# lRomul/sensorium

Hardware: AMD Instinct MI355X
Metric: training clips/sec/GPU (DwiseNeuro fwd+bwd, B=32 T=32 36x64) at 1/2/4/8 GPUs (higher is better)
Workload: dtype bf16

## Files before the change

### include/dwn.h

```cpp
#ifndef DWN_H_
#define DWN_H_
#include <stddef.h>
#include <stdint.h>

#ifdef __cplusplus
extern "C" {
#endif

#define DWN_ABI_VERSION 7
#define DWN_F32 0
#define DWN_BF16 1
#define DWN_F32_AUTO 0
#define DWN_F32_NATIVE 1
#define DWN_F32_SPLIT3 2
#define DWN_BN_EVAL 0
#define DWN_BN_TRAIN 1
#define DWN_BN_FROZEN 2
#define DWN_NREP 32

#define DWN_LD_PLAIN 0
#define DWN_LD_PE 1
#define DWN_LD_BNACT 2
#define DWN_LD_AFFINE2 3
#define DWN_LD_DY3 4
#define DWN_LD_GATE 5
#define DWN_LD_CAT1 6

typedef struct dwn_load_desc {
    const void* p;
    const void* q;
    long long ld;
    const float* v1;
    const float* v2;
    const float* v3;
    const float* v4;
    const float* v5;
    const float* gate;
    const float* gate2;
    int gate_ld;
    int rows_per_sample;
    int act;
    const float* pe_t;
    const float* pe_h;
    const float* pe_w;
    int pT, pH, pW;
    int pe_ld;
    long long ld2;
    int cat_c1, cat_c2;
} dwn_load_desc;

#define DWN_EPI_STORE 0
#define DWN_EPI_READOUT 1
#define DWN_EPI_DG 2
#define DWN_EPI_STORE_CAT 3
#define DWN_EPI_DH3 4

typedef struct dwn_gemm_nn_args {
    dwn_load_desc a;
    int a_kind;
    const void* b; long long ldb;
    void* c; long long ldc;
    int M, N, K;
    int groups;
    double* stats;
    int f32_split;
    int stat_nchan;
    int epi;
    const float* bias; float sp_beta; float* out_nct; int Tn; int n_valid;
    const void* y3; long long ldy3; const float* s3; const float* t3; float* dg; int dg_ld; int rows_per_sample;
    const void* a2; long long a2_ld; int K1;
    long long b_sample_stride; int b_rows_per_sample;
    const float* gate3; const float* dps3; const float* coef3; int coef3_ld;
    int variant;
    const float* sp_beta_dev;
} dwn_gemm_nn_args;
#define DWN_NN_AUTO 0
#define DWN_NN_XL128 1
#define DWN_NN_XL256 2
#define DWN_NN_TILE128 3
#define DWN_NN_KD 4

typedef struct dwn_gemm_tn_args {
    dwn_load_desc p; int p_kind;
    dwn_load_desc q; int q_kind;
    int M, R, Cc;
    float* dw; long long lddw;
    int groups;
    int rows_per_split; int nsplit;
    int R_load;
    int rows_per_sample; int splits_per_sample; long long dw_sample_stride;
    int overwrite;
    int dw_f64;
} dwn_gemm_tn_args;

typedef struct dwn_dw_spatial_fwd_args {
    dwn_load_desc in;
    const float* w;
    void* out;
    int planes, Hin, Win, Hout, Wout, C, stride, ks;
    double* stats;
    int rows_band;
    int impl;
    const void* a0; long long a0_ld; const void* w1; int Cin;
} dwn_dw_spatial_fwd_args;

typedef struct dwn_dw_spatial_bwd_args {
    dwn_load_desc dy;
    dwn_load_desc y1;
    const float* w;
    void* dh1;
    float* dw;
    int planes, Hin, Win, Hout, Wout, C, stride, ks;
    double* stats;
    int rows_band;
    int impl;
    const void* a0; long long a0_ld; const void* w1; int Cin;
} dwn_dw_spatial_bwd_args;

typedef struct dwn_dw_temporal_fwd_args {
    dwn_load_desc in;
    const float* w;
    void* out;
    int B, T, HW, C, kt;
    double* stats;
    const float* z_scale; const float* z_shift; long long* pooled;
} dwn_dw_temporal_fwd_args;

typedef struct dwn_dw_temporal_bwd_args {
    dwn_load_desc dy; int dy_kind;
    dwn_load_desc y2;
    const float* w;
    void* dh2;
    float* dw;
    int B, T, HW, C, kt;
    double* stats;
} dwn_dw_temporal_bwd_args;

typedef struct dwn_bn {
    const float* gamma; const float* beta;
    float* running_mean; float* running_var; long long* num_batches_tracked;
    float* coef;
    float* dgamma; float* dbeta;
} dwn_bn;

typedef struct dwn_stem_args {
    int dtype, training, B, Cin, C0; long long S;
    float eps, momentum;
    const float* x;
    const float* w;
    dwn_bn bn;
    const float *pe_t, *pe_h, *pe_w;
    int T, H, W;
    void* y0;
    void* out;
    const void* dout;
    float* dw;
    void* ws; size_t ws_bytes;
    double* xmom;
} dwn_stem_args;

typedef struct dwn_stem_input_grad_args {
    int dtype, training, B, Cin, C0; long long S;
    const float* w;
// ... 481 lines not shown
```

### sensorium_amd/_lib.py

```python
from __future__ import annotations

import ctypes as C
import os
from pathlib import Path

import torch

_HERE = Path(__file__).resolve().parent
DETERMINISTIC = os.environ.get("DWN_DETERMINISTIC", "0") == "1"
_LIB_NAME = "libdwiseneuro_hip_det.so" if DETERMINISTIC else "libdwiseneuro_hip.so"
LIB_PATH = Path(os.environ["DWN_LIB_PATH"]) if os.environ.get("DWN_LIB_PATH") else _HERE / "csrc" / _LIB_NAME

c_p = C.c_void_p
c_i = C.c_int
c_ll = C.c_longlong
c_f = C.c_float
c_d = C.c_double
c_sz = C.c_size_t

DWN_F32, DWN_BF16 = 0, 1
DWN_NREP = 32
LD_PLAIN, LD_PE, LD_BNACT, LD_AFFINE2, LD_DY3, LD_GATE, LD_CAT1 = 0, 1, 2, 3, 4, 5, 6
EPI_STORE, EPI_READOUT, EPI_DG, EPI_STORE_CAT, EPI_DH3 = 0, 1, 2, 3, 4
NN_AUTO, NN_XL128, NN_XL256, NN_TILE128, NN_KD = 0, 1, 2, 3, 4
F32_AUTO, F32_NATIVE, F32_SPLIT3 = 0, 1, 2
BN_EVAL, BN_TRAIN, BN_FROZEN = 0, 1, 2
FAMILIES = ("pw_fwd", "dws_fwd", "dwt_fwd", "se_pool", "pwl_fwd", "resid_fwd", "resid_bwd", "pwl_dgrad", "pwl_wgrad",
            "bn3_reduce", "dwt_bwd", "dws_bwd", "pw_dgrad", "pw_wgrad", "cortex_fwd", "cortex_bwd", "readout_fwd",
            "readout_bwd")


class LoadDesc(C.Structure):
    _fields_ = [("p", c_p), ("q", c_p), ("ld", c_ll), ("v1", c_p), ("v2", c_p), ("v3", c_p), ("v4", c_p),
                ("v5", c_p), ("gate", c_p), ("gate2", c_p), ("gate_ld", c_i), ("rows_per_sample", c_i),
                ("act", c_i), ("pe_t", c_p), ("pe_h", c_p), ("pe_w", c_p), ("pT", c_i), ("pH", c_i),
                ("pW", c_i), ("pe_ld", c_i), ("ld2", c_ll), ("cat_c1", c_i), ("cat_c2", c_i)]


class GemmNNArgs(C.Structure):
    _fields_ = [("a", LoadDesc), ("a_kind", c_i), ("b", c_p), ("ldb", c_ll), ("c", c_p), ("ldc", c_ll),
                ("M", c_i), ("N", c_i), ("K", c_i), ("groups", c_i), ("stats", c_p),
                ("f32_split", c_i), ("stat_nchan", c_i), ("epi", c_i), ("bias", c_p),
                ("sp_beta", c_f), ("out_nct", c_p), ("Tn", c_i), ("n_valid", c_i), ("y3", c_p), ("ldy3", c_ll),
                ("s3", c_p), ("t3", c_p), ("dg", c_p), ("dg_ld", c_i), ("rows_per_sample", c_i),
                ("a2", c_p), ("a2_ld", c_ll), ("K1", c_i), ("b_sample_stride", c_ll), ("b_rows_per_sample", c_i),
                ("gate3", c_p), ("dps3", c_p), ("coef3", c_p), ("coef3_ld", c_i), ("variant", c_i), ("sp_beta_dev", c_p)]


class GemmTNArgs(C.Structure):
    _fields_ = [("p", LoadDesc), ("p_kind", c_i), ("q", LoadDesc), ("q_kind", c_i), ("M", c_i), ("R", c_i),
                ("Cc", c_i), ("dw", c_p), ("lddw", c_ll), ("groups", c_i), ("rows_per_split", c_i),
                ("nsplit", c_i), ("R_load", c_i), ("rows_per_sample", c_i), ("splits_per_sample", c_i),
                ("dw_sample_stride", c_ll), ("overwrite", c_i), ("dw_f64", c_i)]


class DwSpatialFwdArgs(C.Structure):
    _fields_ = [("inp", LoadDesc), ("w", c_p), ("out", c_p), ("planes", c_i), ("Hin", c_i), ("Win", c_i),
                ("Hout", c_i), ("Wout", c_i), ("C", c_i), ("stride", c_i), ("ks", c_i), ("stats", c_p),
                ("rows_band", c_i), ("impl", c_i),
                ("a0", c_p), ("a0_ld", c_ll), ("w1", c_p), ("Cin", c_i)]


class DwSpatialBwdArgs(C.Structure):
    _fields_ = [("dy", LoadDesc), ("y1", LoadDesc), ("w", c_p), ("dh1", c_p), ("dw", c_p), ("planes", c_i),
                ("Hin", c_i), ("Win", c_i), ("Hout", c_i), ("Wout", c_i), ("C", c_i), ("stride", c_i),
                ("ks", c_i), ("stats", c_p), ("rows_band", c_i), ("impl", c_i),
                ("a0", c_p), ("a0_ld", c_ll), ("w1", c_p), ("Cin", c_i)]


class DwTemporalFwdArgs(C.Structure):
    _fields_ = [("inp", LoadDesc), ("w", c_p), ("out", c_p), ("B", c_i), ("T", c_i), ("HW", c_i), ("C", c_i),
                ("kt", c_i), ("stats", c_p), ("z_scale", c_p), ("z_shift", c_p), ("pooled", c_p)]


class DwTemporalBwdArgs(C.Structure):
    _fields_ = [("dy", LoadDesc), ("dy_kind", c_i), ("y2", LoadDesc), ("w", c_p), ("dh2", c_p), ("dw", c_p),
                ("B", c_i), ("T", c_i), ("HW", c_i), ("C", c_i), ("kt", c_i), ("stats", c_p)]


class BN(C.Structure):
    _fields_ = [("gamma", c_p), ("beta", c_p), ("running_mean", c_p), ("running_var", c_p),
                ("num_batches_tracked", c_p), ("coef", c_p), ("dgamma", c_p), ("dbeta", c_p)]


class StemArgs(C.Structure):
    _fields_ = [("dtype", c_i), ("training", c_i), ("B", c_i), ("Cin", c_i), ("C0", c_i), ("S", c_ll),
                ("eps", c_f), ("momentum", c_f), ("x", c_p), ("w", c_p), ("bn", BN),
                ("pe_t", c_p), ("pe_h", c_p), ("pe_w", c_p), ("T", c_i), ("H", c_i), ("W", c_i),
                ("y0", c_p), ("out", c_p),
                ("dout", c_p), ("dw", c_p), ("ws", c_p), ("ws_bytes", c_sz), ("xmom", c_p)]


class StemInputGradArgs(C.Structure):
    _fields_ = [("dtype", c_i), ("training", c_i), ("B", c_i), ("Cin", c_i), ("C0", c_i), ("S", c_ll),
                ("w", c_p), ("coef", c_p), ("dout", c_p), ("dx", c_p)]


class BlockArgs(C.Structure):
    _fields_ = [("dtype", c_i), ("training", c_i),
                ("B", c_i), ("T", c_i), ("Hin", c_i), ("Win", c_i), ("Hout", c_i), ("Wout", c_i), ("Cin", c_i),
                ("Cmid", c_i), ("Cout", c_i), ("stride", c_i), ("ks", c_i), ("kt", c_i), ("se_r", c_i),
                ("eps", c_f), ("momentum", c_f),
                ("x", c_p), ("out", c_p), ("y1", c_p), ("y2", c_p), ("y3", c_p), ("y4", c_p),
                ("z3", c_p), ("x_has_pe", c_i), ("a0", c_p),
                ("pe_t", c_p), ("pe_h", c_p), ("pe_w", c_p),
                ("out_pe_t", c_p), ("out_pe_h", c_p), ("out_pe_w", c_p),
                ("w_pw", c_p), ("w_dws", c_p), ("w_dwt", c_p), ("w_pwl", c_p), ("se_wr", c_p), ("se_br", c_p),
# ... 169 lines not shown
CORR_STAT_ROWS, CORR_TILE = 8, 16
CORR_MEAN, CORR_SUM = 0, 1
GABOR_GAUSSIAN, GABOR_NONE = 0, 1
BLUR_MAX_RADIUS, BLUR_TAPS_STRIDE, MOMENTS_CHUNK = 16, 33, 4096
MEI_STEP, MEI_PROJECT = 0, 1
MEI_CONTRAST_MAX, MEI_CONTRAST_FIXED = 0, 1
TRIAL_STATE_ROWS, TRIAL_SCORE_ROWS, TRIAL_SUMMARY, TRIAL_TILE = 17, 5, 8, 4
NOISE_BINARY, NOISE_SPARSE = 0, 1
STA_SUMMARY = 8
GAUSS_PARAMS, GAUSS_TABLE = 7, 16
PAIR_TOTAL, PAIR_SIGNAL, PAIR_NOISE = 0, 1, 2
PAIR_TILE, PAIR_KSTEP, PAIR_SUMMARY, PAIR_ROW_STATS = 64, 4, 8, 8
MIX_BOX, MIX_BLEND = 0, 1
VID_U8, VID_F32 = 0, 1

_STRUCTS = {
    "dwn_load_desc": LoadDesc, "dwn_gemm_nn_args": GemmNNArgs, "dwn_gemm_tn_args": GemmTNArgs,
    "dwn_dw_spatial_fwd_args": DwSpatialFwdArgs, "dwn_dw_spatial_bwd_args": DwSpatialBwdArgs,
    "dwn_dw_temporal_fwd_args": DwTemporalFwdArgs, "dwn_dw_temporal_bwd_args": DwTemporalBwdArgs,
    "dwn_bn": BN, "dwn_stem_args": StemArgs, "dwn_block_args": BlockArgs, "dwn_pool_args": PoolArgs,
    "dwn_cortex_args": CortexArgs, "dwn_readout_args": ReadoutArgs, "dwn_tensor_entry": TensorEntry,
    "dwn_clip_src": ClipSrc, "dwn_clip_desc": ClipDesc, "dwn_pw_bwd_args": PwBwdArgs,
    "dwn_dw_spatial_rc_fwd_args": DwSpatialRcFwdArgs, "dwn_stem_input_grad_args": StemInputGradArgs,
    "dwn_guarded_entry": GuardedEntry, "dwn_step_guard": StepGuard, "dwn_gaze_args": GazeArgs,
    "dwn_corr_args": CorrArgs, "dwn_gabor_args": GaborArgs, "dwn_modulator_args": ModulatorArgs,
    "dwn_blur3d_args": Blur3dArgs, "dwn_clip_moments_args": ClipMomentsArgs, "dwn_mei_update_args": MeiUpdateArgs,
    "dwn_trial_desc": TrialDesc, "dwn_trial_group": TrialGroup, "dwn_trial_score_args": TrialScoreArgs,
    "dwn_spatial_gain_args": SpatialGainArgs, "dwn_noise_args": NoiseArgs, "dwn_sta_args": StaArgs,
    "dwn_gauss2d_args": Gauss2dArgs, "dwn_gauss2d_profile_args": Gauss2dProfileArgs,
    "dwn_pair_seg": PairSeg, "dwn_pair_args": PairArgs, "dwn_pair_compare_args": PairCompareArgs,
}

_P = C.POINTER
SYMBOLS = {
    "dwn_abi_version": (c_i, []),
    "dwn_source_hash": (C.c_char_p, []),
    "dwn_sizeof": (c_i, [C.c_char_p]),
    "dwn_last_error": (C.c_char_p, []),
    "dwn_profile_enable": (c_i, [C.c_ulonglong, c_i]),
    "dwn_profile_collect": (c_i, [c_i, _P(c_d), _P(c_ll)]),
    "dwn_gemm_nn": (c_i, [_P(GemmNNArgs), c_i, c_i, c_p]),
    "dwn_gemm_tn": (c_i, [_P(GemmTNArgs), c_i, c_i, c_p]),
    "dwn_dw_spatial_fwd": (c_i, [_P(DwSpatialFwdArgs), c_i, c_i, c_p]),
    "dwn_dw_spatial_bwd": (c_i, [_P(DwSpatialBwdArgs), c_i, c_i, c_p]),
    "dwn_dw_spatial_bwd_rc_supported": (c_i, [_P(DwSpatialBwdArgs), c_i]),
    "dwn_dw_spatial_fwd_rc_supported": (c_i, [_P(DwSpatialFwdArgs), c_i]),
    "dwn_dw_temporal_fwd": (c_i, [_P(DwTemporalFwdArgs), c_i, c_i, c_p]),
    "dwn_dw_temporal_bwd": (c_i, [_P(DwTemporalBwdArgs), c_i, c_i, c_p]),
    "dwn_dw_temporal_wide_fwd": (c_i, [_P(DwTemporalFwdArgs), c_i, c_i, c_p]),
    "dwn_dw_temporal_wide_bwd": (c_i, [_P(DwTemporalBwdArgs), c_i, c_i, c_p]),
    "dwn_bn_finalize": (c_i, [c_p, c_i, c_d, _P(BN), c_i, c_i, c_f, c_f, c_i, c_p]),
    "dwn_bn_bwd_finalize": (c_i, [c_p, c_d, _P(BN), c_p, c_i, c_i, c_p]),
    "dwn_pack_weight": (c_i, [c_p, c_p, c_i, c_i, c_i, c_i, c_i, c_i, c_i, c_i, c_p]),
    "dwn_stem_workspace_bytes": (c_sz, [_P(StemArgs)]),
    "dwn_stem_forward": (c_i, [_P(StemArgs), c_i, c_p]),
    "dwn_stem_backward": (c_i, [_P(StemArgs), c_i, c_p]),
    "dwn_stem_input_grad": (c_i, [_P(StemInputGradArgs), c_i, c_p]),
    "dwn_stem_backward_input": (c_i, [_P(StemArgs), c_p, c_i, c_p]),
    "dwn_block_workspace_bytes": (c_sz, [_P(BlockArgs), c_i]),
    "dwn_block_forward": (c_i, [_P(BlockArgs), c_i, c_p]),
    "dwn_block_backward": (c_i, [_P(BlockArgs), c_i, c_p]),
    "dwn_block_forward_writes": (c_i, [_P(BlockArgs)]),
    "dwn_pool_forward": (c_i, [_P(PoolArgs), c_i, c_p]),
    "dwn_pool_backward": (c_i, [_P(PoolArgs), c_i, c_p]),
    "dwn_cortex_workspace_bytes": (c_sz, [_P(CortexArgs), c_i]),
    "dwn_cortex_forward": (c_i, [_P(CortexArgs), c_i, c_p]),
    "dwn_cortex_backward": (c_i, [_P(CortexArgs), c_i, c_p]),
    "dwn_readout_workspace_bytes": (c_sz, [_P(ReadoutArgs), c_i]),
    "dwn_readout_wt_bytes": (c_sz, [_P(ReadoutArgs)]),
    "dwn_readout_forward": (c_i, [_P(ReadoutArgs), c_i, c_p]),
    "dwn_readout_backward": (c_i, [_P(ReadoutArgs), c_i, c_p]),
    "dwn_poisson_loss_forward": (c_i, [c_p, c_p, c_p, c_ll, c_ll, c_f, c_p, c_i, c_p]),
    "dwn_poisson_loss_backward": (c_i, [c_p, c_p, c_p, c_p, c_ll, c_ll, c_f, c_p, c_i, c_p]),
    "dwn_f64_to_f32": (c_i, [c_p, c_p, c_i, c_i, c_p]),
    "dwn_adamw_ema_multi": (c_i, [c_p, c_i, c_i, c_d, c_d, c_d, c_d, c_d, c_ll, c_d, c_d, c_i, c_p]),
    "dwn_ema_lerp_multi": (c_i, [c_p, c_i, c_i, c_d, c_i, c_p]),
    "dwn_grad_guard_workspace_bytes": (c_sz, [c_i, c_i]),
    "dwn_grad_sumsq_multi": (c_i, [c_p, c_i, c_i, c_d, c_p, c_sz, c_p, c_i, c_p]),
    "dwn_step_guard_finalize": (c_i, [c_p, c_p, c_d, c_i, c_p, c_i, c_p, c_i, c_p]),
    "dwn_adamw_ema_multi_guarded": (c_i, [c_p, c_i, c_i, c_d, c_d, c_d, c_d, c_d, c_d, c_d, c_p, c_i, c_p]),
    "dwn_conv_pw_bn_stats_workspace_bytes": (c_sz, [c_i]),
    "dwn_conv_pw_bn_stats": (c_i, [c_p, c_ll, c_ll, c_p, c_i, c_i, _P(BN), c_f, c_f, c_p, c_p, c_sz, c_i, c_i, c_p]),
    "dwn_pw_bwd_fused_supported": (c_i, [c_i, c_ll, c_i, c_i]),
    "dwn_pw_backward_workspace_bytes": (c_sz, [c_i, c_i, c_i]),
    "dwn_pw_backward": (c_i, [_P(PwBwdArgs), c_i, c_i, c_p]),
    "dwn_dw_spatial_rc_blob_bytes": (c_sz, [c_i, c_i]),
    "dwn_dw_spatial_rc_prep": (c_i, [c_p, c_p, c_p, c_i, c_i, c_p, c_i, c_p]),
    "dwn_dw_spatial_rc_supported": (c_i, [c_i, c_i, c_i, c_i, c_i, c_i, c_i]),
    "dwn_dw_spatial_fwd_rc": (c_i, [_P(DwSpatialRcFwdArgs), c_i, c_p]),
    "dwn_assemble_inputs": (c_i, [c_p, c_i, c_i, c_i, c_i, c_i, c_i, c_f, c_p, c_i, c_p]),
    "dwn_assemble_targets": (c_i, [c_p, c_i, c_i, c_p, c_p, c_i, c_i, c_p, c_i, c_p]),
    "dwn_gaze_shift_forward": (c_i, [_P(GazeArgs), c_i, c_p]),
    "dwn_gaze_shift_backward": (c_i, [_P(GazeArgs), c_i, c_p]),
    "dwn_plane_mean": (c_i, [c_p, c_i, c_i, c_i, c_i, c_i, c_i, c_i, c_p, c_i, c_p]),
    "dwn_corr_ws_bytes": (c_sz, [_P(CorrArgs)]),
    "dwn_corr_moments": (c_i, [_P(CorrArgs), c_i, c_p]),
    "dwn_corr_loss_finalize": (c_i, [_P(CorrArgs), c_i, c_p]),
    "dwn_corr_loss_backward": (c_i, [_P(CorrArgs), c_i, c_p]),
    "dwn_gabor_workspace_bytes": (c_sz, [_P(GaborArgs)]),
    "dwn_gabor_forward": (c_i, [_P(GaborArgs), c_i, c_p]),
    "dwn_gabor_backward": (c_i, [_P(GaborArgs), c_i, c_p]),
    "dwn_modulator_ws_bytes": (c_sz, [_P(ModulatorArgs)]),
    "dwn_modulator_forward": (c_i, [_P(ModulatorArgs), c_i, c_p]),
    "dwn_modulator_backward": (c_i, [_P(ModulatorArgs), c_i, c_p]),
    "dwn_blur3d_ws_bytes": (c_sz, [_P(Blur3dArgs)]),
    "dwn_clip_moments_ws_bytes": (c_sz, [_P(ClipMomentsArgs)]),
    "dwn_blur3d": (c_i, [_P(Blur3dArgs), c_i, c_p]),
    "dwn_clip_moments": (c_i, [_P(ClipMomentsArgs), c_i, c_p]),
    "dwn_mei_update": (c_i, [_P(MeiUpdateArgs), c_i, c_p]),
    "dwn_trial_score_ws_bytes": (c_sz, [_P(TrialScoreArgs)]),
    "dwn_trial_moments": (c_i, [_P(TrialScoreArgs), c_i, c_p]),
    "dwn_trial_score_finalize": (c_i, [_P(TrialScoreArgs), c_i, c_p]),
    "dwn_spatial_gain_ws_bytes": (c_sz, [_P(SpatialGainArgs)]),
    "dwn_spatial_gain_forward": (c_i, [_P(SpatialGainArgs), c_i, c_p]),
    "dwn_spatial_gain_backward": (c_i, [_P(SpatialGainArgs), c_i, c_p]),
    "dwn_pair_ldz": (c_ll, [c_i]),
    "dwn_pair_state_bytes": (c_sz, [_P(PairArgs)]),
    "dwn_pair_ws_bytes": (c_sz, [_P(PairArgs)]),
    "dwn_pair_compare_ws_bytes": (c_sz, [_P(PairCompareArgs)]),
    "dwn_pair_stage": (c_i, [_P(PairArgs), c_i, c_p]),
    "dwn_pair_syrk": (c_i, [_P(PairArgs), c_i, c_p]),
    "dwn_pair_corr_finalize": (c_i, [_P(PairArgs), c_i, c_p]),
    "dwn_pair_compare": (c_i, [_P(PairCompareArgs), c_i, c_p]),
    "dwn_gauss2d_ws_bytes": (c_sz, [_P(Gauss2dArgs)]),
    "dwn_gauss2d_fit": (c_i, [_P(Gauss2dArgs), c_i, c_p]),
    "dwn_gauss2d_profile": (c_i, [_P(Gauss2dProfileArgs), c_i, c_p]),
    "dwn_noise_forward": (c_i, [_P(NoiseArgs), c_i, c_p]),
    "dwn_sta_state_bytes": (c_sz, [_P(StaArgs)]),
    "dwn_sta_ws_bytes": (c_sz, [_P(StaArgs)]),
    "dwn_sta_accumulate": (c_i, [_P(StaArgs), c_i, c_p]),
    "dwn_sta_finalize": (c_i, [_P(StaArgs), c_i, c_p]),
}


class DwnError(RuntimeError):
    pass


HASH_SRCS = ("dwn_api.hip", "dwn_gemm.hip", "dwn_gemm_nn_1.hip", "dwn_gemm_nn_2.hip", "dwn_gemm_nn_3.hip", "dwn_gemm_nn_4.hip", "dwn_gemm_nn_5.hip",
             "dwn_gemm_nn_6.hip", "dwn_gemm_tn.hip", "dwn_pw_bwd.hip", "dwn_gemm_xl.hip", "dwn_gemm_kd.hip", "dwn_dwconv.hip", "dwn_dwrc.hip",
             "dwn_dwbwd.hip", "dwn_dwfwd.hip", "dwn_elementwise.hip", "dwn_data.hip", "dwn_gaze.hip", "dwn_modulator.hip", "dwn_spatial.hip", "dwn_mei.hip", "dwn_rf_fit.hip", "dwn_pairwise.hip", "dwn_trial_score.hip", "dwn_rf.hip", "dwn_corr.hip", "dwn_stim.hip", "dwn_common.h", "dwn_internal.h",
             "dwn_kernels.h", "dwn_launch.h", "dwn_gemm_nn.h", "dwn_gain.h",
             "../../include/dwn.h")


def source_hash() -> str:
    import hashlib
    h = hashlib.sha256()
    for name in HASH_SRCS:
        h.update((_HERE / "csrc" / name).read_bytes())
    return h.hexdigest()[:16]


def _load():
    if not LIB_PATH.exists():
        raise ImportError(
            f"{LIB_PATH} is missing: build it with `python -c 'import __graft_entry__ as g; g.build()'` "
            f"(or `make -C {LIB_PATH.parent}`).  sensorium_amd has no fallback path.")
    lib = C.CDLL(str(LIB_PATH), mode=getattr(os, "RTLD_NOW", 2))
    ab = bool(os.environ.get("DWN_LIB_PATH"))
    for name, (restype, argtypes) in SYMBOLS.items():
        if ab and name in ("dwn_stem_input_grad", "dwn_stem_backward_input", "dwn_grad_guard_workspace_bytes", "dwn_grad_sumsq_multi",
                           "dwn_step_guard_finalize", "dwn_adamw_ema_multi_guarded", "dwn_dw_temporal_wide_fwd",
                           "dwn_dw_temporal_wide_bwd", "dwn_gaze_shift_forward", "dwn_gaze_shift_backward",
                           "dwn_plane_mean", "dwn_corr_ws_bytes", "dwn_corr_moments", "dwn_corr_loss_finalize",
                           "dwn_corr_loss_backward", "dwn_gabor_workspace_bytes", "dwn_gabor_forward",
                           "dwn_gabor_backward", "dwn_modulator_ws_bytes", "dwn_modulator_forward",
                           "dwn_modulator_backward", "dwn_blur3d_ws_bytes", "dwn_clip_moments_ws_bytes", "dwn_blur3d",
                           "dwn_clip_moments", "dwn_mei_update", "dwn_trial_score_ws_bytes", "dwn_trial_moments",
                           "dwn_trial_score_finalize", "dwn_spatial_gain_ws_bytes", "dwn_spatial_gain_forward",
                           "dwn_spatial_gain_backward", "dwn_noise_forward", "dwn_sta_state_bytes", "dwn_sta_ws_bytes",
                           "dwn_sta_accumulate", "dwn_sta_finalize", "dwn_gauss2d_ws_bytes", "dwn_gauss2d_fit",
                           "dwn_gauss2d_profile", "dwn_pair_ldz", "dwn_pair_state_bytes", "dwn_pair_ws_bytes",
                           "dwn_pair_compare_ws_bytes", "dwn_pair_stage", "dwn_pair_syrk", "dwn_pair_corr_finalize",
                           "dwn_pair_compare") and not hasattr(lib, name):
            continue
        fn = getattr(lib, name)
        fn.restype = restype
        fn.argtypes = argtypes
    if lib.dwn_abi_version() != 7 and not (ab and lib.dwn_abi_version() == 6):
        raise ImportError("libdwiseneuro_hip.so ABI version mismatch")
    built, have = lib.dwn_source_hash().decode(), source_hash()
    if built != have and not os.environ.get("DWN_LIB_PATH"):
        raise ImportError(f"{LIB_PATH.name} was built from other sources (binary {built}, tree {have}): rebuild it with "
                          f"`make -C {LIB_PATH.parent}` — binaries are not in git, so what runs must be what is committed")
    for cname, struct in _STRUCTS.items():
        n = lib.dwn_sizeof(cname.encode())
        if n != C.sizeof(struct) and not (ab and (0 < n < C.sizeof(struct) or cname in ("dwn_stem_input_grad_args", "dwn_guarded_entry", "dwn_step_guard", "dwn_gaze_args", "dwn_corr_args", "dwn_gabor_args", "dwn_modulator_args", "dwn_blur3d_args", "dwn_clip_moments_args", "dwn_mei_update_args", "dwn_trial_desc", "dwn_trial_group", "dwn_trial_score_args", "dwn_spatial_gain_args", "dwn_noise_args", "dwn_sta_args", "dwn_gauss2d_args", "dwn_gauss2d_profile_args", "dwn_pair_seg", "dwn_pair_args", "dwn_pair_compare_args"))):
            raise ImportError(f"struct layout mismatch for {cname}: C {n} bytes vs ctypes {C.sizeof(struct)}")
    return lib


lib = _load()


def check(rc: int, what: str = ""):
    if rc != 0:
        msg = lib.dwn_last_error()
        raise DwnError(f"{what} failed (rc={rc}): {msg.decode() if msg else ''}")
```

### sensorium_amd/csrc/dwn_gemm.hip

```cpp
#include "dwn_gemm_nn.h"

template <typename T>
static int launch_nn_d(const GemmNN& g, hipStream_t s) {
    if (g.K % TT<T>::KC != 0) return dwn_set_error(-2, "gemm_nn: K must be a multiple of the 16-byte vector");
    if (g.epi == EPI_READOUT && g.sp_beta_dev) {
        if (g.a_kind == LD_PLAIN) return launch_nn_t<T, LD_PLAIN, EPI_READOUT_LB>(g, s);
        return dwn_set_error(-3, "gemm_nn: the readout epilogue with sp_beta_dev needs a plain loader");
    }
    if (g.epi == EPI_READOUT) {
        if (g.a_kind == LD_BNACT) return launch_nn_t<T, LD_BNACT, EPI_READOUT>(g, s);
        if (g.a_kind == LD_PLAIN) return launch_nn_t<T, LD_PLAIN, EPI_READOUT>(g, s);
        return dwn_set_error(-3, "gemm_nn: unsupported loader for readout epilogue");
    }
    if (g.N % TT<T>::KC != 0) return dwn_set_error(-2, "gemm_nn: N must be a multiple of the 16-byte vector");
    if (g.epi == EPI_DG) {
        if (g.s3 || g.t3) return dwn_set_error(-3, "gemm_nn: the dg epilogue reads the activated z3; s3/t3 must be NULL");
        if (g.a_kind == LD_PLAIN && g.groups == 1) return launch_nn_t<T, LD_PLAIN, EPI_DG>(g, s);
        return dwn_set_error(-3, "gemm_nn: unsupported loader for dg epilogue");
    }
    if (g.epi == EPI_DH3) {
        if (g.a_kind != LD_PLAIN || g.groups != 1 || !g.y3 || !g.gate3 || !g.dps3 || !g.coef3 || g.rows_per_sample <= 0)
            return dwn_set_error(-3, "gemm_nn: the dh3 epilogue needs a plain loader, groups == 1, y3, gate3, dps3, coef3, rows_per_sample");
        return launch_nn_t<T, LD_PLAIN, EPI_DH3>(g, s);
    }
    if (g.epi == EPI_STORE_CAT) {
        if (g.a_kind != LD_PLAIN || g.groups != 1 || g.K1 <= 0 || g.K1 % TT<T>::KC || !g.a2 || !g.bias)
            return dwn_set_error(-3, "gemm_nn: K-concat epilogue needs a plain loader, groups == 1, a2, bias and K1 % vector == 0");
        return launch_nn_t<T, LD_PLAIN, EPI_STORE_CAT>(g, s);
    }
    switch (g.a_kind) {
        case LD_PLAIN: return launch_nn_t<T, LD_PLAIN, EPI_STORE>(g, s);
        case LD_PE: return launch_nn_t<T, LD_PE, EPI_STORE>(g, s);
        case LD_BNACT: return launch_nn_t<T, LD_BNACT, EPI_STORE>(g, s);
        case LD_AFFINE2: return launch_nn_t<T, LD_AFFINE2, EPI_STORE>(g, s);
        case LD_GATE: return launch_nn_t<T, LD_GATE, EPI_STORE>(g, s);
    }
    return dwn_set_error(-3, "gemm_nn: unsupported loader kind");
}

int launch_gemm_nn(const GemmNN& g, int dtype, hipStream_t s) {
    if (g.M <= 0 || g.N <= 0 || g.K <= 0) return 0;
    if (g.b_sample_stride) {
        const int bk = dtype == DWN_BF16 ? 64 : 32;
        if (g.b_rows_per_sample <= 0 || g.b_rows_per_sample % 128 || g.groups != 1 || g.K <= bk)
            return dwn_set_error(-2, "gemm_nn: per-sample weights need b_rows_per_sample % 128 == 0, groups == 1, K > one k-tile");
    }
    if (gemm_nn_kd_eligible(g, dtype)) return launch_gemm_nn_kd(g, s);
    if (gemm_nn_xl_eligible(g, dtype)) return launch_gemm_nn_xl(g, s);
    return dtype == DWN_BF16 ? launch_nn_d<bf16_t>(g, s) : launch_nn_d<float>(g, s);
}
```

### sensorium_amd/csrc/dwn_kernels.h

```cpp
#pragma once
#include "dwn_internal.h"

struct ResGeom {
    int BT, T, Hin, Win, Hout, Wout, Cin, Cout;
    const int* hsrc; const int* wsrc;
    const int* hinv; const int* winv;
};

typedef dwn_tensor_entry TensorListEntry;

struct BnFinJob {
    const double* stats; int stat_c; double count; const float* gamma; const float* beta;
    float* running_mean; float* running_var; long long* nbt; float* coef; int C; int nblocks;
};
struct BnBwdJob { const double* stats; double count; const float* coef; float* dgamma; float* dbeta; float* abc; int C; int nblocks; int frozen; };
int k_bn_finalize_train(BnFinJob j0, BnFinJob j1, float momentum, float eps, hipStream_t s);
int k_bn_bwd_finalize(BnBwdJob j0, BnBwdJob j1, hipStream_t s);
int k_bn_finalize_eval(const float* gamma, const float* beta, const float* rm, const float* rv, float eps,
                       float* coef, int C, hipStream_t s);
int k_bn1_gram_finalize(const double* gram, const float* w1, int E, int Cin, double count, const float* gamma, const float* beta,
                        float* rm, float* rv, long long* nbt, float momentum, float eps, float* coef, double* sc_stats, int dtype,
                        hipStream_t s);
int k_ew_apply(const LoadDesc& d, int kind, void* out, i64 ldo, i64 rows, int C, int dtype, hipStream_t s);
int k_stem_xmom(const float* x, int B, int Cin, i64 S, double* mom, hipStream_t s);
// ... 40 lines not shown
int k_cortex_residual_fwd(const void* y, const void* x, const float* coef, const float* coefsc, const float* dscale,
                          int M, int Tn, int Cin, int C, int groups, void* out, int dtype, hipStream_t s);
int k_cortex_stats(const void* y, const void* x, int M, int Cin, int C, double* stats, double* statssc, int dtype, hipStream_t s);
int k_cortex_bwd_reduce(const void* y, const void* x, const void* dout, const float* gmask, int gmask_ld,
                        const float* coef, const float* coefsc, const float* dscale, int M, int Tn, int Cin, int C,
                        int groups, double* stats, double* statssc, int dtype, hipStream_t s);
int k_cortex_bwd_dy(const void* y, const void* dout, const float* gmask, int gmask_ld, const float* coef,
                    const float* abc, const float* dscale, int M, int Tn, int C, int groups, void* dy, int dtype,
                    hipStream_t s);
int k_cortex_bwd_dx(const void* dxmain, const void* x, const void* dout, const float* gmask, int gmask_ld,
                    const float* abcsc, int M, int Tn, int Cin, int C, void* dx, int dtype, hipStream_t s);
int k_pack_weight(const float* src, void* dst, int groups, int R, int C, int transpose, int Rd, int Cd, int dtype,
                  hipStream_t s);
int k_gate_weights(const float* w, const float* gate, void* dst, int B, int N, int K, int dtype, hipStream_t s);
size_t k_readout_dbeta_parts(int B, int Rp, int groups);
int k_readout_dz(const float* dout, const float* out, float beta, const float* beta_dev, double* part, float* dbeta, int B, int Tn, int n_valid, int Rg, int Rp,
                 int groups, void* dz, float* db, int dtype, hipStream_t s);
int k_poisson_fwd(const float* pred, const float* target, const float* w, i64 per_sample, i64 total, float eps,
                  double* loss, hipStream_t s);
int k_poisson_bwd(const float* pred, const float* target, const float* w, const float* gscale, i64 per_sample,
                  i64 total, float eps, float* dpred, hipStream_t s);
int k_f64_to_f32(const double* src, float* dst, int n, hipStream_t s);
int k_adamw_ema(const TensorListEntry* list, int ntensors, int max_blocks, float decay_w, float omb1, float beta2,
                float omb2, float eps, float step_size, float bc2_sqrt, float ema_decay, float ema_omd,
                float grad_scale, hipStream_t s);
int k_ema_lerp(const TensorListEntry* list, int ntensors, int max_blocks, float decay, float omd, hipStream_t s);
int k_grad_sumsq(const dwn_guarded_entry* list, int ntensors, int max_blocks, double grad_scale, void* ws, double* pair,
                 hipStream_t s);
int k_step_guard_finalize(const double* pair_a, const double* pair_b, double max_norm, int skip_nonfinite,
                          const dwn_guarded_entry* list, int ntensors, dwn_step_guard* guard, hipStream_t s);
int k_adamw_ema_guarded(const dwn_guarded_entry* list, int ntensors, int max_blocks, double lr, double beta1, double beta2,
                        double eps, double weight_decay, double ema_decay, double grad_scale, const dwn_step_guard* guard,
                        hipStream_t s);
int k_fill_f32(float* p, float v, int n, hipStream_t s);
int k_pack_weight_dual(const float* src, void* plain, void* tr, int groups, int R, int C, int Rp, int ldp, int ldt, int dtype,
                       hipStream_t s);
int k_pwl_bwd_reduce(const float* P, const float* gate, const float* W, int B, int K, int N, float* dW, float* dg,
                     hipStream_t s);
int k_assemble_inputs(const dwn_clip_desc* descs, int B, int T, int H0, int W0, int H, int W, float pad, float* x,
                      hipStream_t s);
int k_assemble_targets(const dwn_clip_desc* descs, int B, int T, float* const* targets, const int* n_neurons,
                       int n_mice, int max_neurons, float* mice_weights, hipStream_t s);
int k_zero(void* p, size_t nbytes, hipStream_t s);
int k_gaze_forward(const dwn_gaze_args& a, hipStream_t s);
int k_gaze_backward(const dwn_gaze_args& a, hipStream_t s);
int k_plane_mean(const float* x, int B, int Cin, int T, int H, int W, int c0, int nc, float* mean, hipStream_t s);
size_t k_corr_ws_bytes(int N);
int k_corr_moments(const dwn_corr_args& a, hipStream_t s);
int k_corr_finalize(const dwn_corr_args& a, hipStream_t s);
int k_corr_backward(const dwn_corr_args& a, hipStream_t s);

size_t k_gabor_ws_bytes(const dwn_gabor_args& a);
int k_gabor_forward(const dwn_gabor_args& a, hipStream_t s);
int k_gabor_backward(const dwn_gabor_args& a, hipStream_t s);

size_t k_blur3d_ws_bytes(const dwn_blur3d_args& a);
int k_blur3d(const dwn_blur3d_args& a, hipStream_t s);
size_t k_clip_moments_ws_bytes(const dwn_clip_moments_args& a);
int k_clip_moments(const dwn_clip_moments_args& a, hipStream_t s);
int k_mei_update(const dwn_mei_update_args& a, hipStream_t s);
size_t k_trial_score_ws_bytes(int N);
int k_trial_moments(const dwn_trial_score_args& a, hipStream_t s);
int k_trial_score_finalize(const dwn_trial_score_args& a, hipStream_t s);
size_t k_modulator_ws_bytes(const dwn_modulator_args& a);
int k_modulator_forward(const dwn_modulator_args& a, hipStream_t s);
int k_modulator_backward(const dwn_modulator_args& a, hipStream_t s);
size_t k_spatial_gain_ws_bytes(const dwn_spatial_gain_args& a);
int k_spatial_gain_forward(const dwn_spatial_gain_args& a, hipStream_t s);
int k_spatial_gain_backward(const dwn_spatial_gain_args& a, hipStream_t s);
int k_noise_forward(const dwn_noise_args& a, hipStream_t s);
size_t k_sta_state_bytes(const dwn_sta_args& a);
size_t k_sta_ws_bytes(const dwn_sta_args& a);
int k_sta_accumulate(const dwn_sta_args& a, hipStream_t s);
int k_sta_finalize(const dwn_sta_args& a, hipStream_t s);
size_t k_gauss2d_ws_bytes(const dwn_gauss2d_args& a);
int k_gauss2d_fit(const dwn_gauss2d_args& a, hipStream_t s);
int k_gauss2d_profile(const dwn_gauss2d_profile_args& a, hipStream_t s);
long long k_pair_ldz(int N);
size_t k_pair_compare_ws_bytes(int M);
int k_pair_stage(const dwn_pair_args& a, hipStream_t s);
int k_pair_syrk(const dwn_pair_args& a, hipStream_t s);
int k_pair_corr_finalize(const dwn_pair_args& a, hipStream_t s);
int k_pair_compare(const dwn_pair_compare_args& a, hipStream_t s);
int k_pw_bwd_prep(const float* w1, const float* abc, int E, int C, void* bp, float* gacc, float* r3, int dtype,
                  const float* res_abc, int res_C, hipStream_t s);
size_t pw_wgrad_tacc_floats(int E, int C);
int k_pw_wgrad_fold(const float* tacc, const float* abc, const float* w1, int E, int C, float* dw, int dtype, hipStream_t s);

enum { PREP_ZERO = 0, PREP_FILL = 1, PREP_PACKW = 2, PREP_PACKDW = 3, PREP_BNEVAL = 4 };
#define PREP_MAX_OPS 16
struct PrepOp {
    int kind, nblocks;
    const float* src; void* dst;
    const float* src2; const float* src3; const float* src4;
    long long n;
    float v;
    int R, C, transpose, Rd, Cd;
};
struct PrepArgs {
    int nops;
    PrepOp op[PREP_MAX_OPS];
    PrepArgs() : nops(0) {}
    static int blocks_for(long long n, int cap) { long long b = (n + 255) / 256; return (int)(b > cap ? cap : b); }
    bool zero(void* p, size_t nbytes) {
        if (nbytes == 0) return true;
        if (((size_t)p & 15) || (nbytes & 15) || nops >= PREP_MAX_OPS) return false;
        PrepOp& q = op[nops++]; q = PrepOp(); q.kind = PREP_ZERO; q.dst = p; q.n = (long long)(nbytes / 16); q.nblocks = blocks_for(q.n, 256);
        return true;
    }
    bool fill(float* p, float v, int n) {
        if (n <= 0) return true;
        if (nops >= PREP_MAX_OPS) return false;
        PrepOp& q = op[nops++]; q = PrepOp(); q.kind = PREP_FILL; q.dst = p; q.v = v; q.n = n; q.nblocks = blocks_for(n, 1 << 30);
        return true;
    }
    bool packw(const float* src, void* dst, int groups, int R, int C, int transpose, int Rd, int Cd) {
        if (nops >= PREP_MAX_OPS) return false;
        PrepOp& q = op[nops++]; q = PrepOp(); q.kind = PREP_PACKW; q.src = src; q.dst = dst; q.R = R; q.C = C; q.transpose = transpose;
        q.Rd = Rd; q.Cd = Cd; q.n = (long long)groups * Rd * Cd; q.nblocks = blocks_for(q.n, 1 << 30);
        return true;
    }
    bool packdw(const float* src, float* dst, int C, int taps) {
        if (nops >= PREP_MAX_OPS) return false;
        PrepOp& q = op[nops++]; q = PrepOp(); q.kind = PREP_PACKDW; q.src = src; q.dst = dst; q.C = C; q.R = taps; q.n = (long long)C * taps;
        q.nblocks = blocks_for(q.n, 1 << 30);
        return true;
    }
    bool bneval(const dwn_bn& bn, int C, float eps) {
        if (nops >= PREP_MAX_OPS) return false;
        PrepOp& q = op[nops++]; q = PrepOp(); q.kind = PREP_BNEVAL; q.src = bn.gamma; q.src2 = bn.beta; q.src3 = bn.running_mean;
        q.src4 = bn.running_var; q.dst = bn.coef; q.v = eps; q.n = C; q.C = C; q.nblocks = blocks_for(C, 1 << 30);
        return true;
    }
};
int k_prep(const PrepArgs& pa, int dtype, hipStream_t s);
```

Baseline: 1492.

## Add row-owning persistent GEMM kernel for pwl dgrad with fused dh3 epilogue

Adds a specialised persistent bf16 kernel for the NN GEMM with K=64 and the dh3 epilogue. Each block keeps the whole weight matrix (N up to 448) resident in LDS, owns full output rows, double-buffers the A tile, and fuses the SiLU-gradient, gate scaling and BN statistics into the epilogue. It is selected automatically for N=448 and large M. The aim is to cut repeated weight loads and column tiling overhead for this projection dgrad. In exchange it needs a large LDS footprint with one block per CU, and adds a separate code path to maintain.

```diff
diff --git a/include/dwn.h b/include/dwn.h
--- a/include/dwn.h
+++ b/include/dwn.h
@@ -79,6 +79,8 @@
 #define DWN_NN_XL256 2
 #define DWN_NN_TILE128 3
 #define DWN_NN_KD 4
+#define DWN_NN_ROWS 5
+int dwn_gemm_nn_rows_supported(int dtype, int epi, long long M, int N, int K, int a_kind);
 
 typedef struct dwn_gemm_tn_args {
     dwn_load_desc p; int p_kind;
diff --git a/sensorium_amd/_lib.py b/sensorium_amd/_lib.py
--- a/sensorium_amd/_lib.py
+++ b/sensorium_amd/_lib.py
@@ -22,7 +22,7 @@
 DWN_NREP = 32
 LD_PLAIN, LD_PE, LD_BNACT, LD_AFFINE2, LD_DY3, LD_GATE, LD_CAT1 = 0, 1, 2, 3, 4, 5, 6
 EPI_STORE, EPI_READOUT, EPI_DG, EPI_STORE_CAT, EPI_DH3 = 0, 1, 2, 3, 4
-NN_AUTO, NN_XL128, NN_XL256, NN_TILE128, NN_KD = 0, 1, 2, 3, 4
+NN_AUTO, NN_XL128, NN_XL256, NN_TILE128, NN_KD, NN_ROWS = 0, 1, 2, 3, 4, 5
 F32_AUTO, F32_NATIVE, F32_SPLIT3 = 0, 1, 2
 BN_EVAL, BN_TRAIN, BN_FROZEN = 0, 1, 2
 FAMILIES = ("pw_fwd", "dws_fwd", "dwt_fwd", "se_pool", "pwl_fwd", "resid_fwd", "resid_bwd", "pwl_dgrad", "pwl_wgrad",
@@ -358,6 +358,7 @@
     "dwn_conv_pw_bn_stats_workspace_bytes": (c_sz, [c_i]),
     "dwn_conv_pw_bn_stats": (c_i, [c_p, c_ll, c_ll, c_p, c_i, c_i, _P(BN), c_f, c_f, c_p, c_p, c_sz, c_i, c_i, c_p]),
     "dwn_pw_bwd_fused_supported": (c_i, [c_i, c_ll, c_i, c_i]),
+    "dwn_gemm_nn_rows_supported": (c_i, [c_i, c_i, c_ll, c_i, c_i, c_i]),
     "dwn_pw_backward_workspace_bytes": (c_sz, [c_i, c_i, c_i]),
     "dwn_pw_backward": (c_i, [_P(PwBwdArgs), c_i, c_i, c_p]),
     "dwn_dw_spatial_rc_blob_bytes": (c_sz, [c_i, c_i]),
@@ -414,7 +415,7 @@
 
 
 HASH_SRCS = ("dwn_api.hip", "dwn_gemm.hip", "dwn_gemm_nn_1.hip", "dwn_gemm_nn_2.hip", "dwn_gemm_nn_3.hip", "dwn_gemm_nn_4.hip", "dwn_gemm_nn_5.hip",
-             "dwn_gemm_nn_6.hip", "dwn_gemm_tn.hip", "dwn_pw_bwd.hip", "dwn_gemm_xl.hip", "dwn_gemm_kd.hip", "dwn_dwconv.hip", "dwn_dwrc.hip",
+             "dwn_gemm_nn_6.hip", "dwn_gemm_pwl.hip", "dwn_gemm_tn.hip", "dwn_pw_bwd.hip", "dwn_gemm_xl.hip", "dwn_gemm_kd.hip", "dwn_dwconv.hip", "dwn_dwrc.hip",
              "dwn_dwbwd.hip", "dwn_dwfwd.hip", "dwn_elementwise.hip", "dwn_data.hip", "dwn_gaze.hip", "dwn_modulator.hip", "dwn_spatial.hip", "dwn_mei.hip", "dwn_rf_fit.hip", "dwn_pairwise.hip", "dwn_trial_score.hip", "dwn_rf.hip", "dwn_corr.hip", "dwn_stim.hip", "dwn_common.h", "dwn_internal.h",
              "dwn_kernels.h", "dwn_launch.h", "dwn_gemm_nn.h", "dwn_gain.h",
              "../../include/dwn.h")
@@ -449,7 +450,7 @@
                            "dwn_sta_accumulate", "dwn_sta_finalize", "dwn_gauss2d_ws_bytes", "dwn_gauss2d_fit",
                            "dwn_gauss2d_profile", "dwn_pair_ldz", "dwn_pair_state_bytes", "dwn_pair_ws_bytes",
                            "dwn_pair_compare_ws_bytes", "dwn_pair_stage", "dwn_pair_syrk", "dwn_pair_corr_finalize",
-                           "dwn_pair_compare") and not hasattr(lib, name):
+                           "dwn_pair_compare", "dwn_gemm_nn_rows_supported") and not hasattr(lib, name):
             continue
         fn = getattr(lib, name)
         fn.restype = restype
diff --git a/sensorium_amd/csrc/dwn_gemm.hip b/sensorium_amd/csrc/dwn_gemm.hip
--- a/sensorium_amd/csrc/dwn_gemm.hip
+++ b/sensorium_amd/csrc/dwn_gemm.hip
@@ -1,4 +1,5 @@
 #include "dwn_gemm_nn.h"
+#include "dwn_kernels.h"
 
 template <typename T>
 static int launch_nn_d(const GemmNN& g, hipStream_t s) {
@@ -45,6 +46,9 @@
         if (g.b_rows_per_sample <= 0 || g.b_rows_per_sample % 128 || g.groups != 1 || g.K <= bk)
             return dwn_set_error(-2, "gemm_nn: per-sample weights need b_rows_per_sample % 128 == 0, groups == 1, K > one k-tile");
     }
+    if (gemm_nn_rows_eligible(g, dtype)) return launch_gemm_nn_rows(g, s);
+    if (g.variant == DWN_NN_ROWS)
+        return dwn_set_error(-2, "gemm_nn: DWN_NN_ROWS needs bf16, a plain loader, the dh3 epilogue with its tensors, groups == 1, K == 64, N % 64 == 0, N <= 448");
     if (gemm_nn_kd_eligible(g, dtype)) return launch_gemm_nn_kd(g, s);
     if (gemm_nn_xl_eligible(g, dtype)) return launch_gemm_nn_xl(g, s);
     return dtype == DWN_BF16 ? launch_nn_d<bf16_t>(g, s) : launch_nn_d<float>(g, s);
diff --git a/sensorium_amd/csrc/dwn_gemm_pwl.hip b/sensorium_amd/csrc/dwn_gemm_pwl.hip
--- /dev/null
+++ b/sensorium_amd/csrc/dwn_gemm_pwl.hip
@@ -0,0 +1,263 @@
+#include "dwn_gemm_nn.h"
+#include "dwn_kernels.h"
+
+#ifndef PWL_ROWS_AUTO
+#define PWL_ROWS_AUTO 1
+#endif
+#define PWL_ROWS_AUTO_MIN_M 589824
+
+constexpr int PWL_BN = 64, PWL_ROWB = 128, PWL_THREADS = 512;
+constexpr int PWL_MAX_NCT = 7;
+
+template <int NCT> struct PwlGeom {
+    static constexpr int N = NCT * PWL_BN;
+    static constexpr int CPR = N / 8;
+    static constexpr int RL = PWL_THREADS / CPR;
+    static constexpr int P = (64 + RL - 1) / RL;
+    static constexpr int BM = RL * P;
+    static constexpr int RB = (BM + 15) / 16;
+    static constexpr int CROW = N * 2 + 16;
+    static constexpr int SA_BYTES = RB * 16 * PWL_ROWB;
+    static constexpr int RED_BYTES = RL * 2 * N * (int)sizeof(float);
+    static constexpr int SC_BYTES = BM * CROW > RED_BYTES ? BM * CROW : RED_BYTES;
+    static constexpr int A_CH = (RB * 16 * 8 + PWL_THREADS - 1) / PWL_THREADS;
+    static constexpr size_t LDS = (size_t)N * PWL_ROWB + 2 * SA_BYTES + SC_BYTES;
+};
+
+template <int NCT>
+__global__ __launch_bounds__(PWL_THREADS, 1) void pwl_dgrad_rows_kernel(const GemmNN g) {
+    using T = bf16_t;
+    using Geo = PwlGeom<NCT>;
+    constexpr int KC = 8, ROWB = PWL_ROWB, N = Geo::N, CPR = Geo::CPR, RL = Geo::RL, P = Geo::P, BM = Geo::BM, RB = Geo::RB;
+    constexpr int CROW = Geo::CROW, A_CH = Geo::A_CH;
+    extern __shared__ __attribute__((aligned(16))) unsigned char smem_pwl[];
+    unsigned char* const sB = smem_pwl;
+    unsigned char* const sA = sB + N * ROWB;
+    unsigned char* const sC = sA + 2 * Geo::SA_BYTES;
+
+    const int tid = threadIdx.x;
+    const int ntm = (g.M + BM - 1) / BM;
+    const int G = (int)gridDim.x;
+    const int lid = ((int)blockIdx.x & 7) * (G >> 3) + ((int)blockIdx.x >> 3);
+    const int mt_beg = (int)((i64)lid * ntm / G);
+    const int mt_end = (int)((i64)(lid + 1) * ntm / G);
+    if (mt_beg >= mt_end) { DET_EXIT(); return; }
+
+    const T* Ap = reinterpret_cast<const T*>(g.a.p);
+    const T* Bp = reinterpret_cast<const T*>(g.b);
+    const T* Yp = reinterpret_cast<const T*>(g.y3);
+    T* Cp = reinterpret_cast<T*>(g.c);
+    const int Mlast = g.M - 1;
+
+    for (int c = tid; c < N * 8; c += PWL_THREADS) {
+        const int row = c >> 3, kc = c & 7;
+        *reinterpret_cast<uint4*>(sB + row * ROWB + ((kc ^ (row & 7)) << 4)) = *reinterpret_cast<const uint4*>(Bp + (i64)row * g.ldb + kc * KC);
+    }
+    static_assert(A_CH <= 2, "dy4 chunks per thread");
+    uint4 ra0, ra1 = make_uint4(0, 0, 0, 0);
+    auto a_src = [&](int m0, int c) -> const uint4* {
+        c = c < RB * 16 * 8 ? c : RB * 16 * 8 - 1;
+        int m = m0 + (c >> 3);
+        m = m < Mlast ? m : Mlast;
+        return reinterpret_cast<const uint4*>(Ap + (i64)m * g.a.ld + (c & 7) * KC);
+    };
+    auto a_dst = [&](unsigned char* dst, int c) -> uint4* {
+        c = c < RB * 16 * 8 ? c : RB * 16 * 8 - 1;
+        const int row = c >> 3, kc = c & 7;
+        return reinterpret_cast<uint4*>(dst + row * ROWB + ((kc ^ (row & 7)) << 4));
+    };
+    auto load_a = [&](int m0) {
+        ra0 = *a_src(m0, tid);
+        if constexpr (A_CH > 1) ra1 = *a_src(m0, tid + PWL_THREADS);
+    };
+    auto store_a = [&](unsigned char* dst) {
+        *a_dst(dst, tid) = ra0;
+        if constexpr (A_CH > 1) *a_dst(dst, tid + PWL_THREADS) = ra1;
+    };
+    load_a(mt_beg * BM);
+    store_a(sA);
+
+    const int wave = tid >> 6, lane = tid & 63;
+    const int lr = lane & 15, lg = lane >> 4;
+    const int ech = tid % CPR, erl = tid / CPR;
+    const bool eact = erl < RL;
+    const int ncol = ech * KC;
+    const int erow = eact ? erl : RL - 1;
+
+    float sc3[KC], sh3[KC], gt3[KC], gp3[KC], st0[KC], st1[KC];
+    ld_coef<KC>(g.coef3 + ncol, sc3);
+    ld_coef<KC>(g.coef3 + (i64)g.coef3_ld + ncol, sh3);
+#pragma unroll
+    for (int i = 0; i < KC; ++i) { st0[i] = 0.f; st1[i] = 0.f; gt3[i] = 0.f; gp3[i] = 0.f; }
+    int gb = -1;
+
+    uint4 yv[P];
+    auto y_src = [&](int m0, int p) -> const uint4* {
+        int m = m0 + erow + RL * p;
+        m = m < Mlast ? m : Mlast;
+        return reinterpret_cast<const uint4*>(Yp + (i64)m * g.ldy3 + ncol);
+    };
+#pragma unroll
+    for (int p = 0; p < P; ++p) yv[p] = *y_src(mt_beg * BM, p);
+    int buf = 0;
+    nn_lds_barrier();
+
+    auto tile = [&](const int mt, auto fast_c) {
+        constexpr bool fast = decltype(fast_c)::value;
+        const int m0 = mt * BM;
+        const unsigned char* tA = sA + buf * Geo::SA_BYTES;
+        load_a(m0 + BM);
+        if constexpr (fast) {
+            const int b = m0 / g.rows_per_sample;
+            if (b != gb) {
+                gb = b;
+                ld_coef<KC>(g.gate3 + (i64)b * g.dg_ld + ncol, gt3);
+                ld_coef<KC>(g.dps3 + (i64)b * g.dg_ld + ncol, gp3);
+            }
+        }
+        if (wave < NCT) {
+            uint4 bfr[2][4];
+#pragma unroll
+            for (int kb = 0; kb < 2; ++kb)
+#pragma unroll
+                for (int j = 0; j < 4; ++j) {
+                    const int row = wave * PWL_BN + j * 16 + lr;
+                    bfr[kb][j] = *reinterpret_cast<const uint4*>(sB + row * ROWB + (((kb * 4 + lg) ^ (row & 7)) << 4));
+                }
+#pragma unroll
+            for (int rb = 0; rb < RB; ++rb) {
+                const int trow = rb * 16 + lr;
+                f32x4_t acc[4];
+#pragma unroll
+                for (int j = 0; j < 4; ++j) acc[j] = f32x4_t{0.f, 0.f, 0.f, 0.f};
+#pragma unroll
+                for (int kb = 0; kb < 2; ++kb) {
+                    const uint4 af = *reinterpret_cast<const uint4*>(tA + trow * ROWB + (((kb * 4 + lg) ^ (trow & 7)) << 4));
+#pragma unroll
+                    for (int j = 0; j < 4; ++j) Mma<T>::run(bfr[kb][j], af, acc[j]);
+                }
+                if ((rb + 1) * 16 <= BM || trow < BM) {
+#pragma unroll
+                    for (int j = 0; j < 4; ++j) {
+                        const int col = wave * PWL_BN + j * 16 + lg * 4;
+                        uint2 v;
+                        v.x = pk_bf16(acc[j][0], acc[j][1]);
+                        v.y = pk_bf16(acc[j][2], acc[j][3]);
+                        *reinterpret_cast<uint2*>(sC + trow * CROW + col * 2) = v;
+                    }
+                }
+            }
+        }
+        nn_lds_barrier();
+#pragma unroll
+        for (int p = 0; p < P; ++p) {
+            const int row = erow + RL * p;
+            const int m = m0 + row;
+            const uint4 raw = *reinterpret_cast<const uint4*>(sC + row * CROW + ech * 16);
+            float v[KC], y[KC], dh[KC];
+            unpack16<T>(raw, v);
+            unpack16<T>(yv[p], y);
+            yv[p] = *y_src(m0 + BM, p);
+            if constexpr (fast) {
+#pragma unroll
+                for (int i = 0; i < KC; ++i) dh[i] = fmaf(y[i], sc3[i], sh3[i]);
+                silu_grad_n<KC>(dh, dh);
+#pragma unroll
+                for (int i = 0; i < KC; ++i) dh[i] = fmaf(v[i], gt3[i], gp3[i]) * dh[i];
+                const uint4 packed = pack16<T>(dh);
+                *reinterpret_cast<uint4*>(Cp + (i64)m * g.ldc + ncol) = packed;
+                if (g.stats) {
+                    float r[KC];
+                    unpack16<T>(packed, r);
+#pragma unroll
+                    for (int i = 0; i < KC; ++i) { st0[i] += r[i]; st1[i] = fmaf(r[i], y[i], st1[i]); }
+                }
+            } else {
+                if (eact && m < g.M) {
+                    const int b = m / g.rows_per_sample;
+                    if (b != gb) {
+                        gb = b;
+                        ld_coef<KC>(g.gate3 + (i64)b * g.dg_ld + ncol, gt3);
+                        ld_coef<KC>(g.dps3 + (i64)b * g.dg_ld + ncol, gp3);
+                    }
+#pragma unroll
+                    for (int i = 0; i < KC; ++i) dh[i] = fmaf(y[i], sc3[i], sh3[i]);
+                    silu_grad_n<KC>(dh, dh);
+#pragma unroll
+                    for (int i = 0; i < KC; ++i) dh[i] = fmaf(v[i], gt3[i], gp3[i]) * dh[i];
+                    const uint4 packed = pack16<T>(dh);
+                    *reinterpret_cast<uint4*>(Cp + (i64)m * g.ldc + ncol) = packed;
+                    if (g.stats) {
+                        float r[KC];
+                        unpack16<T>(packed, r);
+#pragma unroll
+                        for (int i = 0; i < KC; ++i) { st0[i] += r[i]; st1[i] = fmaf(r[i], y[i], st1[i]); }
+                    }
+                }
+            }
+        }
+        buf ^= 1;
+        store_a(sA + buf * Geo::SA_BYTES);
+        nn_lds_barrier();
+    };
+    for (int mt = mt_beg; mt < mt_end; ++mt) {
+        const int m0_ = mt * BM;
+        const bool fast = m0_ + BM <= g.M && (m0_ / g.rows_per_sample == (m0_ + BM - 1) / g.rows_per_sample);
+        if (fast) tile(mt, std::true_type{}); else tile(mt, std::false_type{});
+    }
+
+    if (g.stats) {
+        float* const red = reinterpret_cast<float*>(sC);
+        if (eact) {
+            float mu3[KC], is3[KC];
+            ld_coef<KC>(g.coef3 + 2 * (i64)g.coef3_ld + ncol, mu3);
+            ld_coef<KC>(g.coef3 + 3 * (i64)g.coef3_ld + ncol, is3);
+#pragma unroll
+            for (int i = 0; i < KC; ++i) {
+                red[erl * (2 * N) + ncol + i] = st0[i];
+                red[erl * (2 * N) + N + ncol + i] = is3[i] * fmaf(-mu3[i], st0[i], st1[i]);
+            }
+        }
+        nn_lds_barrier();
+        DET_ENTER();
+        for (int c = tid; c < 2 * N; c += PWL_THREADS) {
+            float s = 0.f;
+            for (int r = 0; r < RL; ++r) s += red[r * (2 * N) + c];
+            stat_add(g.stats, (int)(blockIdx.x % DWN_NREP), g.stat_nchan, c / N, c % N, s);
+        }
+    }
+    DET_EXIT();
+}
+
+template <int NCT>
+static int launch_pwl_rows_n(const GemmNN& g, hipStream_t s) {
+    const i64 ntm = ((i64)g.M + PwlGeom<NCT>::BM - 1) / PwlGeom<NCT>::BM;
+    return launch_resident(pwl_dgrad_rows_kernel<NCT>, PWL_THREADS, PwlGeom<NCT>::LDS, 1, 1, ntm, true, s, g);
+}
+
+int dwn_gemm_nn_rows_supported(int dtype, int epi, long long M, int N, int K, int a_kind) {
+    return dtype == DWN_BF16 && epi == DWN_EPI_DH3 && a_kind == DWN_LD_PLAIN && M >= 1 && M <= 0x7fffffffLL && N >= PWL_BN &&
+           N % PWL_BN == 0 && N <= PWL_MAX_NCT * PWL_BN && K == 64;
+}
+
+bool gemm_nn_rows_eligible(const GemmNN& g, int dtype) {
+    if (g.variant != DWN_NN_AUTO && g.variant != DWN_NN_ROWS) return false;
+    if (!dwn_gemm_nn_rows_supported(dtype, g.epi, g.M, g.N, g.K, g.a_kind)) return false;
+    if (g.groups != 1 || g.b_sample_stride || !g.y3 || !g.gate3 || !g.dps3 || !g.coef3 || g.rows_per_sample <= 0) return false;
+    if ((g.a.ld | g.ldb | g.ldc | g.ldy3) % 8 != 0 || g.dg_ld % 4 != 0 || g.coef3_ld % 4 != 0) return false;
+    if (g.variant == DWN_NN_ROWS) return true;
+    return PWL_ROWS_AUTO != 0 && g.N == 448 && g.M >= PWL_ROWS_AUTO_MIN_M;
+}
+
+int launch_gemm_nn_rows(const GemmNN& g, hipStream_t s) {
+    switch (g.N / PWL_BN) {
+        case 1: return launch_pwl_rows_n<1>(g, s);
+        case 2: return launch_pwl_rows_n<2>(g, s);
+        case 3: return launch_pwl_rows_n<3>(g, s);
+        case 4: return launch_pwl_rows_n<4>(g, s);
+        case 5: return launch_pwl_rows_n<5>(g, s);
+        case 6: return launch_pwl_rows_n<6>(g, s);
+        case 7: return launch_pwl_rows_n<7>(g, s);
+    }
+    return dwn_set_error(-2, "gemm_nn: the row-owning dh3 kernel takes N = 64 .. 448 in steps of 64");
+}
diff --git a/sensorium_amd/csrc/dwn_kernels.h b/sensorium_amd/csrc/dwn_kernels.h
--- a/sensorium_amd/csrc/dwn_kernels.h
+++ b/sensorium_amd/csrc/dwn_kernels.h
@@ -146,6 +146,8 @@
 int k_pair_syrk(const dwn_pair_args& a, hipStream_t s);
 int k_pair_corr_finalize(const dwn_pair_args& a, hipStream_t s);
 int k_pair_compare(const dwn_pair_compare_args& a, hipStream_t s);
+bool gemm_nn_rows_eligible(const GemmNN& g, int dtype);
+int launch_gemm_nn_rows(const GemmNN& g, hipStream_t s);
 int k_pw_bwd_prep(const float* w1, const float* abc, int E, int C, void* bp, float* gacc, float* r3, int dtype,
                   const float* res_abc, int res_C, hipStream_t s);
 size_t pw_wgrad_tacc_floats(int E, int C);
```

Result: no change. 1482 (-0.6%).
